# sanjita2911/CS230-distributed-machine-learning

Hardware: AMD Instinct MI355X
Metric: CV-fits/sec (whole node), 256-pt RF GridSearchCV on 1M×100 tabular (higher is better)
Workload: dtype fp32; 1 GPU; model=RandomForestClassifier, global_batch=20, parallelism=task1, rows=1000000, features=100, grid_points=256, cv=5, cands_per_rank_step=4

## Files before the change

### cs230_distributed_machine_learning_amd/csrc/kernels/forest.hip

```cpp
#include <hip/hip_runtime.h>
#include <stdint.h>
#include <math.h>
#include <type_traits>
#include <algorithm>
#include <stdio.h>
#include <stdlib.h>
#include <string.h>
#include "forest_common.h"
#include "wave_ops.h"

#ifndef DML_RPT_BLOCK
#define DML_RPT_BLOCK 1
#endif
#if DML_RPT_BLOCK < 1 || DML_RPT_BLOCK > 4
#error "DML_RPT_BLOCK must be 1..4"
#endif
#ifndef DML_BLOCK_NT
#define DML_BLOCK_NT 128
#endif
template <int MODE> constexpr int block_nt() { return MODE == 1 ? DML_BLOCK_NT : 256; }
#ifndef DML_NODES_WPE
#define DML_NODES_WPE 4
#endif
#ifndef DML_EVAL_NOINLINE
#define DML_EVAL_ATTR __attribute__((always_inline))
#else
#define DML_EVAL_ATTR
#endif
#ifndef DML_PART_U2
#define DML_PART_U2 4
#endif
#ifndef DML_KGL_LARGE
#define DML_KGL_LARGE 16
#endif
#ifndef DML_KGW_LARGE
#define DML_KGW_LARGE 32
#endif
#ifndef DML_LARGE_STASH
#define DML_LARGE_STASH 0
#endif
#ifndef DML_PART_KEEP
#define DML_PART_KEEP 2
#endif
#ifndef DML_NODES_WPE_WAVE
#define DML_NODES_WPE_WAVE 4
#endif
#ifndef DML_NODES_WPE_WAVE_MAX
#define DML_NODES_WPE_WAVE_MAX 8
#endif
#ifndef DML_KGMAX_BLOCK
#define DML_KGMAX_BLOCK 16
#endif
#ifndef DML_BLOCK_STREAM_ONLY
#define DML_BLOCK_STREAM_ONLY 1
#endif
#ifndef DML_NODES_WPE_REG
#define DML_NODES_WPE_REG 2
#endif
#ifndef DML_NODES_WPE_MC
#define DML_NODES_WPE_MC 2
#endif
#ifndef DML_SUB_SEG_REG
#define DML_SUB_SEG_REG 1
#endif
#ifndef DML_KGMAX_WAVE
#define DML_KGMAX_WAVE 4
#endif
#ifndef DML_WAVE_HIST32
#define DML_WAVE_HIST32 1
#endif
#ifndef DML_KGMAX_WAVE32
#define DML_KGMAX_WAVE32 5
#endif
#ifndef DML_ROW_WINDOWS
#define DML_ROW_WINDOWS 1
#endif
#ifndef DML_WAVE_WIN_ROWS
#define DML_WAVE_WIN_ROWS 4
#endif
#ifndef DML_GINI_PF
#define DML_GINI_PF 1
#endif
#ifndef DML_EVAL_PAIRS
#define DML_EVAL_PAIRS 0
#endif
#ifndef DML_WAVE_PREFETCH
#define DML_WAVE_PREFETCH 12
#endif
#ifndef DML_LARGE_NODE_FAST
#define DML_LARGE_NODE_FAST 1
#endif
#if DML_LARGE_NODE_FAST
// ... 880 lines not shown
    if (!PK && !c.packed) return pack_bin32(c.ycls[r.wd], boot_weight(s, r.wd));
    return pack_bin32((int)(r.wd >> (c.rbits + 4)), (r.wd >> c.rbits) & 15u);
  } else {
    return word_payload<MODE, PK>(c, s, ty, r.wd);
  }
}

template <int MODE>
__device__ __forceinline__ void hist_add_unit(typename HT<MODE>::T* hj, int b, const typename PLT<MODE>::T& pl,
                                              int wo) {
  if constexpr (MODE == 2) {
    atomicAdd((uint32_t*)hj + b, 1u);
    atomicAdd(&hj[wo + b], pl.wy);
  }
}

constexpr int kPackShift = 52;
constexpr unsigned long long kPackBias = 1ull << 39;
template <int MODE>
__device__ __forceinline__ void hist_add_packed(typename HT<MODE>::T* hj, int b, const typename PLT<MODE>::T& pl,
                                                int wo) {
  if constexpr (MODE == 2) atomicAdd(&hj[wo + b], (1ull << kPackShift) + ((unsigned long long)pl.wy + kPackBias));
}
__device__ __forceinline__ uint32_t pack_count(unsigned long long v) { return (uint32_t)(v >> kPackShift); }
__device__ __forceinline__ unsigned long long pack_wy(unsigned long long v) {
  return (v & ((1ull << kPackShift) - 1)) - ((v >> kPackShift) << 39);
}

template <int MODE>
__device__ __forceinline__ void hist_add_wy(typename HT<MODE>::T* hj, int b, const typename PLT<MODE>::T& pl,
                                            int wo) {
  if constexpr (MODE == 2) atomicAdd(&hj[wo + b], pl.wy);
}

template <int MODE, int RP = 3, class CT = typename HT<MODE>::T, class PL = typename PLT<MODE>::T>
__device__ __forceinline__ void hist_add(CT* hj, const Ctx& c, int b, const PL& pl) {
#ifdef DML_X2_ATOMIC
  if constexpr (MODE == 1) atomicAdd(&hj[b], (CT)(pl * (PL)((uint32_t)c.n >> 31)));
#endif
  if constexpr (MODE == 2) {
    atomicAdd(&hj[b], pl.wr);
    atomicAdd(&hj[256 + b], pl.wy);
    if (RP == 3) atomicAdd(&hj[512 + b], pl.wyy);
    return;
  }
  if constexpr (MODE == 0) {
    atomicAdd(&hj[(int)(uint32_t)pl * 256 + b], (uint32_t)(pl >> 32));
    atomicAdd(&hj[c.C * 256 + b], 1u);
  } else if constexpr (MODE == 1) {
    atomicAdd(&hj[b], (CT)pl);
  }
}

template <int NT, int MODE, int FC, bool H32 = false>
__global__ __launch_bounds__(NT) __attribute__((amdgpu_waves_per_eu(MODE == 2 ? DML_NODES_WPE_REG : (MODE == 0 ? DML_NODES_WPE_MC : (NT == 64 ? DML_NODES_WPE_WAVE : DML_NODES_WPE)), (MODE == 1 && NT == 64) ? DML_NODES_WPE_WAVE_MAX : 8))) void k_nodes(Ctx c, int tier, int set_cur,
                                                                                                   int pair_base, int stage_base) {
  static_assert(!H32 || (MODE == 1 && NT == 64), "the narrow word is the binary wave tier's");
  using CT = typename std::conditional<H32, uint32_t, typename HT<MODE>::T>::type;
  constexpr bool PK = FC >= 0;
  constexpr int NW = NT / 64;
  constexpr int RPT = NT == 64 ? 4 : DML_RPT_BLOCK;
  static_assert(RPT >= 1 && RPT <= 4, "RPT");
  static_assert(2 * RPT * (NT / 64) <= 32, "Scratch::wcnt too small for this NT x RPT");
  constexpr int KGMAX = NT == 64 ? (H32 ? DML_KGMAX_WAVE32 : DML_KGMAX_WAVE) : DML_KGMAX_BLOCK;
  extern __shared__ __attribute__((aligned(16))) unsigned char smem[];
  PH_BEGIN
  const OpenNode on = c.open[set_cur][tier][blockIdx.x];
  const NodeSpec s = spec_of<FC>(c, on.tree);
  const int tid = threadIdx.x, lane = tid & 63, wid = tid >> 6;
  const int d = c.d;
  const int KG = min(NT == 64 ? c.kg_wave : c.kg_block, KGMAX);
  const int slack = NT == 64 ? c.slack_wave : 0;
  const int span = hist_planes(MODE, c.CH) * 256;
  const FusedLayout FL = fused_layout(KG, span, (int)sizeof(CT), c.CH);
  CT* hist = (CT*)(smem + FL.hist);
  int16_t* feats = (int16_t*)(smem + FL.feats);
  double* rg = (double*)(smem + FL.rg);
  int* rb = (int*)(smem + FL.rb);
  int* rn = (int*)(smem + FL.rn);
  double* rleft = (double*)(smem + FL.rleft);
  double* rmid = (double*)(smem + FL.rmid);
  double* best_left = (double*)(smem + FL.best_left);
  double* pvs = (double*)(smem + FL.pvs);
  double* rvs = (double*)(smem + FL.rvs);
  Scratch* sc = (Scratch*)(smem + FL.sc);

  for (int i = tid; i < KG * span; i += NT) hist[i] = (CT)0;
  if (tid < c.VC) pvs[tid] = c.node_val[(int64_t)on.node * c.VC + tid];
  if (tid == 0) {
    sc->best_gain = -INFINITY; sc->best_feat = -1; sc->best_bin = -1;
    sc->nonconst = 0; sc->pos = 0; sc->first = 1; sc->last = 0; sc->best_j = -1;
    sc->best_pos = 1 << 30; sc->scr_n = 0;
    sc->W = c.tree_W[on.tree];
    sc->best_mid = 0.0;
    sc->lo = (FC < 0 && c.nbound) ? c.nbound[2 * (int64_t)on.node] : -INFINITY;
    sc->hi = (FC < 0 && c.nbound) ? c.nbound[2 * (int64_t)on.node + 1] : INFINITY;
  }
  const FeatPerm fp = feat_perm(on.key, d);
  const uint32_t* rows = c.rows_cur + on.start;
  const float* ty = tree_y(c, s);
  const int cnt = on.count;
  const bool reg_rows = (NT > 64 && DML_BLOCK_STREAM_ONLY) ? false : (H32 || cnt <= NT * RPT);
  uint32_t rrow[RPT], rbin[RPT];
  using PL = typename std::conditional<H32, uint32_t, typename PLT<MODE>::T>::type;
  PL rpl[RPT];
  PRaw rpr[RPT];
  auto load_rows = [&](int base) {
#pragma unroll
    for (int u = 0; u < RPT; ++u) {
      const int r = base + tid + NT * u;
      rrow[u] = r < cnt ? rows[r] : 0xFFFFFFFFu;
    }
  };
  auto fetch_rows = [&]() {
#pragma unroll
    for (int u = 0; u < RPT; ++u) rpr[u] = payload_fetch<MODE, PK>(c, ty, rrow[u]);
  };
  auto finish_rows = [&]() {
#pragma unroll
    for (int u = 0; u < RPT; ++u)
      rpl[u] = rrow[u] != 0xFFFFFFFFu ? payload_finish<MODE, PK, PL>(c, s, ty, rpr[u]) : PL{};
  };
  if (reg_rows) load_rows(0);
#pragma unroll
  for (int u = 0; u < RPT; ++u) rbin[u] = 0;
  __syncthreads();
  PH(0)
  if (reg_rows) fetch_rows();
  const int k = s.max_features;
  uint32_t pk[KGMAX];
  constexpr int KPRE = (NT == 64 && RPT == 4) ? DML_WAVE_PREFETCH : 0;
  uint32_t pre[KPRE > 0 ? KPRE : 1];
  int npre = 0;
  if constexpr (KPRE > 0) {
    if (reg_rows) {
      npre = min(KPRE, min(k + slack, d));
      if (DML_ROW_WINDOWS && DML_WAVE_WIN_ROWS > 0 && npre >= 8 && d <= 112 && (c.ld & 15) == 0 && c.ld >= 112 &&
          (((uintptr_t)c.Xb) & 15) == 0) {
        typedef uint32_t v32u __attribute__((ext_vector_type(32)));
        int fdw[KPRE], fsh[KPRE];
#pragma unroll
        for (int q = 0; q < KPRE; ++q) {
          const int f = __builtin_amdgcn_readfirstlane(q < npre ? feature_at(fp, q, d) : 0);
          fdw[q] = f >> 2;
          fsh[q] = (f & 3) * 8;
          pre[q] = 0u;
        }
        constexpr int WR = DML_WAVE_WIN_ROWS > 0 ? DML_WAVE_WIN_ROWS : 1;
#pragma unroll
        for (int u0 = 0; u0 < RPT; u0 += WR) {
          v32u w[WR];
#pragma unroll
          for (int uu = 0; uu < WR; ++uu) {
            const uint32_t r = rrow[u0 + uu];
// ... 30 lines not shown
      for (int q = 0; q < KPRE; ++q) {
        uint32_t v = 0;
#pragma unroll
        for (int u = 0; u < RPT; ++u) v |= raw[q][u] << (8 * u);
        pre[q] = v;
      }
      }
    }
  }
  if (reg_rows) finish_rows();
  while (true) {
    const int pos = __builtin_amdgcn_readfirstlane(sc->pos), nonconst = __builtin_amdgcn_readfirstlane(sc->nonconst);
    if (nonconst >= k || pos >= d) break;
    const int g = min(KG, min(k - nonconst + slack, d - pos));
    if (tid < g) feats[tid] = (int16_t)feature_at(fp, pos + tid, d);
    __syncthreads();
    PH(1)
    if (KPRE > 0 && reg_rows && pos + g <= npre) {
#pragma unroll
      for (int q = 0; q < (KPRE > 0 ? KPRE : 1); ++q) {
        if (q >= pos && q < pos + g) {
          CT* hj = hist + (q - pos) * span;
#pragma unroll
          for (int u = 0; u < RPT; ++u)
            if (rrow[u] != 0xFFFFFFFFu) hist_add<MODE>(hj, c, (int)((pre[q] >> (8 * u)) & 0xFFu), rpl[u]);
        }
      }
    } else
    if (!reg_rows && RPT == 1) {
      constexpr uint32_t INV = 0xFFFFFFFFu;
      auto run = [&](auto Gc) {
        constexpr int G = decltype(Gc)::value;
        int fj[G];
#pragma unroll
        for (int j = 0; j < G; ++j) fj[j] = __builtin_amdgcn_readfirstlane((int)feats[j < g ? j : 0]);
        auto row_at = [&](int r) -> uint32_t {
          const uint32_t v = rows[min(r, cnt - 1)];
          return r < cnt ? v : INV;
        };
        auto gather = [&](uint32_t r, uint32_t* b) {
          const uint8_t* xr = c.Xb + (int64_t)(r != INV ? (r & c.rmask) : 0u) * c.ld;
#pragma unroll
          for (int j = 0; j < G; ++j) b[j] = (uint32_t)xr[fj[j]];
#ifdef DML_X2_GATHER
#pragma unroll
          for (int j = 0; j < G; ++j) b[j] |= (uint32_t)xr[fj[j] + ((uint32_t)c.n >> 31)];
#endif
        };
        auto consume = [&](int base, bool valid, const uint32_t* b, const PRaw& pr) {
          if (NT > 64 && pos == 0 && valid) {
            uint32_t w4[4] = {0u, 0u, 0u, 0u};
#pragma unroll
            for (int j = 0; j < G && j < 16; ++j) w4[j >> 2] |= (j < g ? b[j] & 0xFFu : 0u) << (8 * (j & 3));
            *(uint4*)(c.bscr + (on.start + base + tid) * 16) = make_uint4(w4[0], w4[1], w4[2], w4[3]);
          }
          if (valid) {
            const PL pl = payload_finish<MODE, PK, PL>(c, s, ty, pr);
#pragma unroll
            for (int j = 0; j < G; ++j)
              if (j < g) hist_add<MODE>(hist + j * span, c, (int)b[j], pl);
          }
        };
        uint32_t rA = row_at(tid), rB = row_at(NT + tid);
        uint32_t bA[G], bB[G];
        gather(rA, bA);
        PRaw pA = payload_fetch<MODE, PK>(c, ty, rA), pB;
        bool vA = rA != INV, vB = false;
        for (int base = 0; base < cnt; base += 2 * NT) {
          rA = row_at(base + 2 * NT + tid);
          gather(rB, bB);
          pB = payload_fetch<MODE, PK>(c, ty, rB);
          vB = rB != INV;
          consume(base, vA, bA, pA);
          rB = row_at(base + 3 * NT + tid);
          gather(rA, bA);
          pA = payload_fetch<MODE, PK>(c, ty, rA);
          vA = rA != INV;
          consume(base + NT, vB, bB, pB);
        }
      };
      auto runw = [&](auto Gc) {
        constexpr int G = decltype(Gc)::value;
        typedef uint32_t v32u __attribute__((ext_vector_type(32)));
        int fdw[G], fsh[G];
#pragma unroll
        for (int j = 0; j < G; ++j) {
          const int f = __builtin_amdgcn_readfirstlane((int)feats[j < g ? j : 0]);
          fdw[j] = f >> 2;
          fsh[j] = (f & 3) * 8;
        }
        auto row_at = [&](int r) -> uint32_t {
          const uint32_t v = rows[min(r, cnt - 1)];
          return r < cnt ? v : INV;
        };
        auto load_win = [&](uint32_t r, v32u& w) {
          const uint4* xr = (const uint4*)(c.Xb + (int64_t)(r != INV ? (r & c.rmask) : 0u) * c.ld);
#pragma unroll
          for (int k = 0; k < 7; ++k) {
            const uint4 q = xr[k];
            w[4 * k] = q.x; w[4 * k + 1] = q.y; w[4 * k + 2] = q.z; w[4 * k + 3] = q.w;
          }
        };
        constexpr int NPK = (G + 3) / 4;
        auto extract = [&](const v32u& w, uint32_t* b) {
#pragma unroll
          for (int q = 0; q < NPK; ++q) b[q] = 0u;
#pragma unroll
          for (int j = 0; j < G; ++j) b[j >> 2] |= (j < g ? (w[fdw[j]] >> fsh[j]) & 0xFFu : 0u) << (8 * (j & 3));
        };
        auto consume = [&](int base, bool valid, const uint32_t* b, const PRaw& pr) {
          if (NT > 64 && pos == 0 && valid)
            *(uint4*)(c.bscr + (on.start + base + tid) * 16) =
                make_uint4(b[0], NPK > 1 ? b[NPK > 1 ? 1 : 0] : 0u, NPK > 2 ? b[NPK > 2 ? 2 : 0] : 0u,
                           NPK > 3 ? b[NPK > 3 ? 3 : 0] : 0u);
          if (valid) {
            const PL pl = payload_finish<MODE, PK, PL>(c, s, ty, pr);
#pragma unroll
            for (int j = 0; j < G; ++j)
              if (j < g) hist_add<MODE>(hist + j * span, c, (int)((b[j >> 2] >> (8 * (j & 3))) & 0xFFu), pl);
          }
        };
        v32u win;
        uint32_t bA[NPK], bB[NPK];
        uint32_t rA = row_at(tid), rB = row_at(NT + tid);
        load_win(rA, win);
        PRaw pA = payload_fetch<MODE, PK>(c, ty, rA), pB;
        extract(win, bA);
        bool vA = rA != INV, vB = false;
        for (int base = 0; base < cnt; base += 2 * NT) {
          load_win(rB, win);
          pB = payload_fetch<MODE, PK>(c, ty, rB);
          rA = row_at(base + 2 * NT + tid);
          consume(base, vA, bA, pA);
          extract(win, bB);
          vB = rB != INV;
          load_win(rA, win);
          pA = payload_fetch<MODE, PK>(c, ty, rA);
          rB = row_at(base + 3 * NT + tid);
          consume(base + NT, vB, bB, pB);
          extract(win, bA);
          vA = rA != INV;
        }
      };
      if (DML_ROW_WINDOWS && NT > 64 && pos == 0 && g >= 8 && d <= 112 && (c.ld & 15) == 0 && c.ld >= 112 &&
          (((uintptr_t)c.Xb) & 15) == 0) {
        switch (g) {
          case 8: runw(std::integral_constant<int, (8 < KGMAX ? 8 : KGMAX)>{}); break;
          case 9: runw(std::integral_constant<int, (9 < KGMAX ? 9 : KGMAX)>{}); break;
          case 10: runw(std::integral_constant<int, (10 < KGMAX ? 10 : KGMAX)>{}); break;
          case 11: runw(std::integral_constant<int, (11 < KGMAX ? 11 : KGMAX)>{}); break;
          case 12: runw(std::integral_constant<int, (12 < KGMAX ? 12 : KGMAX)>{}); break;
          default: runw(std::integral_constant<int, KGMAX>{}); break;
        }
      } else
      switch (g) {
#define DML_G_CASE(N) case N: run(std::integral_constant<int, (N < KGMAX ? N : KGMAX)>{}); break;
        DML_G_CASE(1) DML_G_CASE(2) DML_G_CASE(3) DML_G_CASE(4) DML_G_CASE(5) DML_G_CASE(6) DML_G_CASE(7)
        DML_G_CASE(8) DML_G_CASE(9) DML_G_CASE(10) DML_G_CASE(11) DML_G_CASE(12) DML_G_CASE(13) DML_G_CASE(14)
        DML_G_CASE(15)
#undef DML_G_CASE
        default: run(std::integral_constant<int, KGMAX>{}); break;
      }
    } else
    for (int base = 0; base < cnt; base += NT * RPT) {
      if (!reg_rows) { load_rows(base); fetch_rows(); }
      uint32_t bins[KGMAX][RPT];
#pragma unroll
      for (int j = 0; j < KGMAX; ++j) {
        if (j < g) {
          const int64_t f = feats[j];
#pragma unroll
          for (int u = 0; u < RPT; ++u)
            bins[j][u] = rrow[u] != 0xFFFFFFFFu ? (uint32_t)c.Xb[(int64_t)(rrow[u] & c.rmask) * c.ld + f] : 0u;
        }
      }
      if (!reg_rows) finish_rows();
#pragma unroll
      for (int j = 0; j < KGMAX; ++j) {
        if (j < g) {
          CT* hj = hist + j * span;
#pragma unroll
          for (int u = 0; u < RPT; ++u)
            if (rrow[u] != 0xFFFFFFFFu) hist_add<MODE>(hj, c, (int)bins[j][u], rpl[u]);
        }
      }
      if (NT > 64 && !reg_rows && pos == 0) {
#pragma unroll
        for (int u = 0; u < RPT; ++u)
          if (rrow[u] != 0xFFFFFFFFu) {
            uint32_t w4[4] = {0u, 0u, 0u, 0u};
#pragma unroll
            for (int j = 0; j < KGMAX && j < 16; ++j)
              if (j < g) w4[j >> 2] |= (bins[j][u] & 0xFFu) << (8 * (j & 3));
            *(uint4*)(c.bscr + (on.start + base + tid + NT * u) * 16) = make_uint4(w4[0], w4[1], w4[2], w4[3]);
          }
      }
      if (NT == 64 && !reg_rows && pos < 16) {
#pragma unroll
        for (int u = 0; u < RPT; ++u)
          if (rrow[u] != 0xFFFFFFFFu) {
            uint8_t* slot = c.bscr + (on.start + base + tid + NT * u) * 16;
#pragma unroll
            for (int j = 0; j < KGMAX; ++j)
              if (j < g && pos + j < 16) slot[pos + j] = (uint8_t)bins[j][u];
          }
      }
      if (reg_rows) {
#pragma unroll
        for (int j = 0; j < KGMAX; ++j)
        {
          uint32_t v = 0;
#pragma unroll
          for (int u = 0; u < RPT; ++u) v |= bins[j][u] << (8 * u);
          pk[j] = j < g ? v : 0u;
        }
      }
    }
    __syncthreads();
    PH(2)
    int j0 = wid;
#if !defined(DML_X2_EVAL) && DML_EVAL_PAIRS
    if constexpr (MODE == 1 && (DML_EVAL_PAIRS == 1 || (DML_EVAL_PAIRS == 2) == (NT == 64))) {
      const double* cw = tree_cw<FC>(c, on.tree);
      if (gini_pf_ok(s, cwk(cw, 0), cwk(cw, 1)))
        for (; j0 + NW < g; j0 += 2 * NW) {
          if (mono_of<FC>(c, s, feats[j0]) != 0 || mono_of<FC>(c, s, feats[j0 + NW]) != 0) break;
          eval_gini_pf<2, NW, CT>(hist + j0 * span, span, s, lane, rg + j0, rb + j0, rn + j0, rleft + j0 * c.CH, c.CH, true,
                              cwk(cw, 0), cwk(cw, 1));
          if (lane == 0) { rmid[j0] = 0.0; rmid[j0 + NW] = 0.0; }
        }
    }
#endif
    for (int j = j0; j < g; j += NW) {
#ifdef DML_X2_EVAL
      eval_feature<MODE, 3, CT>(hist + j * span, c.C, c.CH, s, lane, rg + j, rb + j, rn + j, rleft + j * c.CH, false,
                         tree_cw<FC>(c, on.tree), &c.rq, MonoQ{mono_of<FC>(c, s, feats[j]), sc->lo, sc->hi}, rmid + j);
      wave_lds_sync();
#endif
      eval_feature<MODE, 3, CT>(hist + j * span, c.C, c.CH, s, lane, rg + j, rb + j, rn + j, rleft + j * c.CH, true,
                         tree_cw<FC>(c, on.tree), &c.rq, MonoQ{mono_of<FC>(c, s, feats[j]), sc->lo, sc->hi}, rmid + j);
    }
    __syncthreads();
    PH(3)
    if (wid == 0) {
      const int nc0 = sc->nonconst;
      const bool isnc = lane < g && rn[lane] != 0;
      const uint64_t m = __ballot(isnc);
// ... 24 lines not shown
#pragma unroll
        for (int q = 0; q < (KPRE > 0 ? KPRE : 1); ++q)
          if (q == pos + bj) sel = pre[q];
      } else {
#pragma unroll
        for (int j = 0; j < KGMAX; ++j)
          if (j == bj) sel = pk[j];
      }
      if (bj >= 0)
#pragma unroll
        for (int u = 0; u < RPT; ++u) rbin[u] = (sel >> (8 * u)) & 0xFFu;
    }
  }
  if (tid == 0) {
    int base = pair_base + 2 * (int)blockIdx.x;
    NodeRec leaf; leaf.split = -1; leaf.left = -1;
    c.nodes[base] = leaf;
    c.nodes[base + 1] = leaf;
    if (!(sc->best_feat >= 0 && accept_split_v(c, s, pvs, sc->W, best_left))) {
      base = -1;
      c.stage[2 * (stage_base + (int64_t)blockIdx.x)].tier = -1;
      c.stage[2 * (stage_base + (int64_t)blockIdx.x) + 1].tier = -1;
    } else {
      {
        double* lv = c.node_val + (int64_t)base * c.VC;
        for (int q = 0; q < c.VC; ++q) {
          rvs[q] = pvs[q] - best_left[q];
          lv[q] = best_left[q];
          lv[c.VC + q] = rvs[q];
        }
        NodeRec rec; rec.split = pack_split(sc->best_feat, sc->best_bin); rec.left = base;
        c.nodes[on.node] = rec;
        mono_children<FC>(c, on.node, base, mono_of<FC>(c, s, sc->best_feat), sc->best_mid);
      }
    }
    sc->base = base;
    sc->nl = base >= 0 ? (int)best_left[c.CH - 1] : 0;
  }
  __syncthreads();
  PH(5)
  const int base = sc->base;
  if (base < 0) { PH_END(NT == 64 ? 0 : 1) return; }
  const int feat = sc->best_feat, bin = sc->best_bin, nl = sc->nl;
  constexpr int RT = NT > 64 ? 64 : 1;
  if (tid == 0)
    stage_child<FC>(c, s, on.tree, base, on.start, nl, on.depth + 1, child_key(on.key, 0),
                2 * (stage_base + (int64_t)blockIdx.x), best_left);
  if (tid == RT)
    stage_child<FC>(c, s, on.tree, base + 1, on.start + nl, cnt - nl, on.depth + 1, child_key(on.key, 1),
                2 * (stage_base + (int64_t)blockIdx.x) + 1, rvs);
#ifdef DML_X2_PART
  for (int rep_ = 0; rep_ < 2; ++rep_) {
#endif
  if (NT > 64 && !reg_rows && cnt <= 128 * NT && (size_t)((cnt + 63) / 64) * 12 <= (size_t)KG * span * sizeof(CT)) {
    uint64_t* lflag = (uint64_t*)hist;
    int* loff = (int*)(lflag + ((cnt + 63) / 64));
    const int ngrp = (cnt + 63) / 64;
    const int bjs = __builtin_amdgcn_readfirstlane((sc->best_pos < sc->scr_n) ? sc->best_pos : -1);
    const int fsplit = __builtin_amdgcn_readfirstlane(feat), bsplit = __builtin_amdgcn_readfirstlane(bin);
    constexpr int U = 4;
    constexpr int KR = DML_PART_KEEP;
    static_assert(DML_PART_U2 == U, "pass 2 walks the positions of pass 1");
    uint32_t rk[KR > 0 ? KR : 1][U];
#pragma unroll
    for (int q = 0; q < (KR > 0 ? KR : 1); ++q)
#pragma unroll
      for (int u = 0; u < U; ++u) rk[q][u] = 0u;
    for (int p0 = 0, q = 0; p0 < cnt; p0 += U * NT, ++q) {
      uint32_t bv[U];
#pragma unroll
      for (int u = 0; u < U; ++u) {
        const int p = min(p0 + u * NT + tid, cnt - 1);
        const uint32_t r = (KR > 0 || bjs < 0) ? rows[p] : 0u;
        if (bjs >= 0) {
          bv[u] = c.bscr[(on.start + p) * 16 + bjs];
        } else {
          bv[u] = c.Xb[(int64_t)(r & c.rmask) * c.ld + fsplit];
        }
#pragma unroll
        for (int qq = 0; qq < KR; ++qq)
          if (qq == q) rk[qq][u] = r;
      }
#pragma unroll
      for (int u = 0; u < U; ++u) {
        const int p = p0 + u * NT + tid;
        const uint64_t m = __ballot(p < cnt && (int)bv[u] <= bsplit);
        if (lane == 0 && p - lane < cnt) lflag[(p - lane) >> 6] = m;
      }
    }
    __syncthreads();
    {
      const int g0 = 2 * tid, g1 = 2 * tid + 1;
      const int c0 = g0 < ngrp ? __popcll(lflag[g0]) : 0, c1 = g1 < ngrp ? __popcll(lflag[g1]) : 0;
      const int incl = wave::incl_scan<int>(c0 + c1);
      if (lane == 63) sc->wcnt[wid] = incl;
      __syncthreads();
      int wbase = 0;
      for (int w = 0; w < wid; ++w) wbase += sc->wcnt[w];
      const int ex = wbase + incl - (c0 + c1);
      if (g0 < ngrp) loff[g0] = ex;
      if (g1 < ngrp) loff[g1] = ex + c0;
    }
    __syncthreads();
    constexpr int U2 = DML_PART_U2;
    for (int p0 = tid, q = 0; p0 < cnt; p0 += U2 * NT, ++q) {
      uint32_t rr[U2];
      if (q < KR) {
#pragma unroll
        for (int qq = 0; qq < KR; ++qq)
          if (qq == q)
#pragma unroll
            for (int u = 0; u < U2; ++u) rr[u] = rk[qq][u];
      } else {
#pragma unroll
        for (int u = 0; u < U2; ++u) rr[u] = rows[min(p0 + u * NT, cnt - 1)];
      }
#pragma unroll
      for (int u = 0; u < U2; ++u) {
        const int p = p0 + u * NT;
        if (p >= cnt) break;
        const int q = p >> 6;
        const uint64_t m = lflag[q];
        const int lft = __popcll(m & ((1ull << (p & 63)) - 1ull));
        const bool left = (m >> (p & 63)) & 1ull;
        const int l0 = loff[q];
        c.rows_next[on.start + (left ? l0 + lft : nl + (q * 64 - l0) + ((p & 63) - lft))] = rr[u];
      }
    }
  } else {
  uint32_t* out = c.rows_next + on.start;
  int baseL = 0, baseR = 0;
  constexpr uint32_t INVR = 0xFFFFFFFFu;
  auto prow = [&](int r) -> uint32_t { return r < cnt ? rows[r] : INVR; };
  const int bj_scr = (!reg_rows && sc->best_pos < sc->scr_n) ? sc->best_pos : -1;
  auto pbin = [&](int p, uint32_t r) -> uint32_t {
    if (r == INVR) return 0u;
    if (bj_scr >= 0) return (uint32_t)c.bscr[(on.start + p) * 16 + bj_scr];
    return (uint32_t)c.Xb[(int64_t)(r & c.rmask) * c.ld + feat];
  };
  uint32_t nrow = INVR, nbin = 0, frow = INVR;
  if (!reg_rows && RPT == 1) {
    rrow[0] = prow(tid);
    rbin[0] = pbin(tid, rrow[0]);
    nrow = prow(NT + tid);
  }
  for (int cb = 0; cb < cnt; cb += NT * RPT) {
    if (!reg_rows) {
      if constexpr (RPT == 1) {
        nbin = pbin(cb + NT + tid, nrow);
        frow = prow(cb + 2 * NT + tid);
      } else {
        load_rows(cb);
#pragma unroll
        for (int u = 0; u < RPT; ++u)
          rbin[u] = rrow[u] == 0xFFFFFFFFu ? 0u
                  : bj_scr >= 0 ? (uint32_t)c.bscr[(on.start + cb + tid + NT * u) * 16 + bj_scr]
                                : (uint32_t)c.Xb[(int64_t)(rrow[u] & c.rmask) * c.ld + feat];
      }
    }
    uint64_t ml[RPT], mr[RPT];
#pragma unroll
    for (int u = 0; u < RPT; ++u) {
      const bool valid = rrow[u] != 0xFFFFFFFFu;
      const bool left = valid && (int)rbin[u] <= bin;
      ml[u] = __ballot(left);
      mr[u] = __ballot(valid && !left);
    }
    int offL[RPT], offR[RPT], totL = 0, totR = 0;
    if constexpr (NW == 1) {
#pragma unroll
      for (int u = 0; u < RPT; ++u) {
        offL[u] = totL; offR[u] = totR;
        totL += __popcll(ml[u]); totR += __popcll(mr[u]);
      }
    } else {
      if (lane == 0)
#pragma unroll
        for (int u = 0; u < RPT; ++u) {
          sc->wcnt[u * NW + wid] = __popcll(ml[u]);
          sc->wcnt[RPT * NW + u * NW + wid] = __popcll(mr[u]);
        }
      __syncthreads();
#pragma unroll
      for (int u = 0; u < RPT; ++u) {
        int l = 0, r = 0, lb = 0, rbb = 0;
        for (int w = 0; w < NW; ++w) {
          const int cl = sc->wcnt[u * NW + w], cr = sc->wcnt[RPT * NW + u * NW + w];
          if (w < wid) { lb += cl; rbb += cr; }
          l += cl; r += cr;
        }
        offL[u] = totL + lb; offR[u] = totR + rbb;
        totL += l; totR += r;
      }
      __syncthreads();
    }
#pragma unroll
    for (int u = 0; u < RPT; ++u) {
      const bool valid = rrow[u] != 0xFFFFFFFFu;
      if (!valid) continue;
      if ((int)rbin[u] <= bin) out[baseL + offL[u] + lane_prefix(ml[u])] = rrow[u];
      else out[nl + baseR + offR[u] + lane_prefix(mr[u])] = rrow[u];
    }
    baseL += totL; baseR += totR;
    if (!reg_rows && RPT == 1) { rrow[0] = nrow; rbin[0] = nbin; nrow = frow; }
  }
  }
#ifdef DML_X2_PART
  }
#endif
// ... 1926 lines not shown
  t_lane = lane;
  return kLanes;
}

__global__ void k_test_wave_prims(const uint32_t* in, uint32_t* out) {
  const int lane = threadIdx.x;
  const uint32_t v = in[blockIdx.x * 64 + lane];
  uint32_t* o = out + (size_t)blockIdx.x * 64 * 11;
  o[0 * 64 + lane] = wave::bitonic64(v, lane);
  o[1 * 64 + lane] = wave::incl_scan<uint32_t>(v);
  o[2 * 64 + lane] = wave::xor32<1>(v, lane);
  o[3 * 64 + lane] = wave::xor32<2>(v, lane);
  o[4 * 64 + lane] = wave::xor32<4>(v, lane);
  o[5 * 64 + lane] = wave::xor32<8>(v, lane);
  o[6 * 64 + lane] = wave::xor32<16>(v, lane);
  o[7 * 64 + lane] = wave::xor32<32>(v, lane);
  double g = (double)(v % 97u);
  int idx = lane;
  wave::argmax(g, idx, lane);
  o[8 * 64 + lane] = (uint32_t)idx;
  o[9 * 64 + lane] = (uint32_t)wave::shift_down1<int>((int)v, lane, -1);
  o[10 * 64 + lane] = (uint32_t)wave::min_u64(((uint64_t)v << 32) | (uint32_t)lane, lane);
}

struct PredictArgs;
extern "C" int dml_forest_predict_fit(const PredictArgs* a, int32_t f, hipStream_t st);

extern "C" {

int dml_forest_phase_stats(unsigned long long* out) {
#ifdef DML_PHASE_PROF
  if (hipMemcpyFromSymbol(out, HIP_SYMBOL(g_phase), sizeof(unsigned long long) * 32) != hipSuccess) return 1;
  unsigned long long z[32] = {0};
  if (hipMemcpyToSymbol(HIP_SYMBOL(g_phase), z, sizeof(z)) != hipSuccess) return 1;
  return 0;
#else
  (void)out;
  return 2;
#endif
}

int dml_test_wave_prims(const uint32_t* in, uint32_t* out, int64_t nblocks, hipStream_t st) {
  k_test_wave_prims<<<(unsigned)nblocks, 64, 0, st>>>(in, out);
  return hipGetLastError() == hipSuccess ? 0 : 1;
}

const char* dml_forest_last_error(int* line) {
  if (line) *line = g_last_err_line;
  return hipGetErrorString(g_last_err);
}

int dml_forest_wave_hist32() { return DML_WAVE_HIST32 != 0 ? 1 : 0; }
int dml_forest_large_stash() { return DML_LARGE_STASH != 0 ? 1 : 0; }
int dml_forest_sizeof_treespec() { return (int)sizeof(TreeSpec); }
int dml_forest_sizeof_args() { return (int)sizeof(ForestArgs); }
int dml_forest_sizeof_node() { return (int)sizeof(NodeRec); }

int64_t dml_forest_workspace_bytes(const ForestArgs* a) {
  Layout L = plan(a);
  return (int64_t)(L.total + align_up((size_t)a->rows_total * 4, 256));
}

int dml_forest_count(ForestArgs* a, hipStream_t st) {
  Ctx c{};
  c.n = (int)a->n; c.roles = (const uint8_t*)a->roles; c.specs = (const TreeSpec*)a->specs;
  c.active_count = (int32_t*)a->active_count;
  HIP_OK(hipMemsetAsync(c.active_count, 0, a->T * 4, st));
  dim3 grid((unsigned)((a->n + 1023) / 1024), (unsigned)((a->T + kCntG - 1) / kCntG));
  k_count_active<<<grid, 256, 0, st>>>(c, (int)a->T);
  HIP_OK(hipGetLastError());
  return 0;
}

}

template <int MODE>
static int build_impl(ForestArgs* a, hipStream_t st) {
  constexpr bool REG = MODE == 2;
  constexpr int GM = MODE == 2 ? 2 : 0;
  constexpr int FCX = REG ? kMSE : kGini;
  Layout L = plan(a);
  if ((size_t)a->workspace_bytes < (size_t)dml_forest_workspace_bytes(a)) return 2;
  Ctx c = make_ctx(a, L);
  const bool fast = a->fast_crit == FCX + 1 && c.packed;
  const bool big = MODE == 1 && a->bigsub_max > 0;
  if (big && (a->bigsub_max > 256 || a->wave_max > a->bigsub_max || a->sub_cache_d <= 0 || a->mono || a->n_classes != 2))
    return 12;
  if (big) c.bigsub_max = (int)a->bigsub_max;
  const size_t lds_big = big ? big_layout((int)a->bigsub_max, (int)a->sub_cache_d).total + 16 : 0;
  uint32_t* rows_a = (uint32_t*)(((unsigned char*)a->workspace) + L.total);
  c.rows_cur = rows_a;
  int32_t* h = pinned_counters();
  if (!h) return 3;
  const bool reg = REG;
  if (!reg && (a->n_classes < 1 || a->n_classes > kMaxClasses)) return 5;
  if (a->d > 32767) return 6;

  HIP_OK(hipMemsetAsync(c.counters, 0, kNumCounters * 4, st));
  HIP_OK(hipMemsetAsync(c.cursors, 0, a->T * 4, st));
  HIP_OK(hipMemsetAsync(c.node_val, 0, (size_t)a->T * c.VC * 8, st));
  if (reg) HIP_OK(hipMemsetAsync(c.rsum, 0, (size_t)a->T * 3 * 8, st));
  k_init_counters<<<1, 1, 0, st>>>(c);
  dim3 gfill((unsigned)((a->n + 1023) / 1024), (unsigned)a->T);
  if (reg) k_fill_active<true><<<gfill, 256, 0, st>>>(c);
  else k_fill_active<false><<<gfill, 256, 0, st>>>(c);
  k_roots<<<(unsigned)((a->T + 255) / 256), 256, 0, st>>>(c);
// ... 271 lines not shown
```

### cs230_distributed_machine_learning_amd/csrc/kernels/forest_common.h

```cpp
#pragma once
#include <stdint.h>

#if defined(__HIPCC__)
#include <hip/hip_runtime.h>
#define DML_HD __host__ __device__ __forceinline__
#define DML_HDM __host__ __device__ __forceinline__
#else
#include <math.h>
#define DML_HD static inline
#define DML_HDM inline
#endif

namespace dml {

constexpr int kBins = 256;
constexpr int kPoisTable = 12;
constexpr int kMaxClasses = 64;

enum Criterion : int32_t { kGini = 0, kEntropy = 1, kMSE = 2, kPoisson = 3, kMAE = 4, kFriedman = 5 };

struct TreeSpec {
  uint64_t seed;
  int32_t split;
  int32_t fit;
// ... 78 lines not shown
  p.m3 = ((uint32_t)h3 | 1u) & p.mask; p.a3 = (uint32_t)(h3 >> 32) & p.mask;
  if (p.mask == 1u) { p.m1 = p.m2 = p.m3 = 1u; }
  return p;
}

DML_HD uint32_t feat_perm_step(const FeatPerm& p, uint32_t x) {
  x = (x * p.m1 + p.a1) & p.mask;
  x ^= x >> p.sh;
  x = (x * p.m2 + p.a2) & p.mask;
  x ^= x >> p.sh;
  x = (x * p.m3 + p.a3) & p.mask;
  x ^= x >> p.sh;
  return x;
}

DML_HD int feature_at(const FeatPerm& p, int k, int d) {
  uint32_t x = feat_perm_step(p, (uint32_t)k);
  while (x >= (uint32_t)d) x = feat_perm_step(p, x);
  return (int)x;
}

constexpr uint64_t kPackMask21 = (1ull << 21) - 1ull;
constexpr int kPackMaxRows = 131072;
DML_HD uint64_t pack_bin(int cls, uint32_t w) {
  return (cls == 0 ? (uint64_t)w : ((uint64_t)w << 21)) | (1ull << 42);
}

constexpr int kRowWeightBits = 4;
constexpr int kPack32MaxRows = 255;
constexpr int kPack32MaxWeight = 1 << kRowWeightBits;
constexpr uint32_t kPack32Mask12 = (1u << 12) - 1u;
static_assert(kPoisTable < kPack32MaxWeight, "a bootstrap weight must fit the row word's weight field");
static_assert(kPack32MaxWeight * kPack32MaxRows < 4096, "a 255-row node's class weight must fit 12 bits");
static_assert(kPack32MaxRows < 256, "a 255-row node's row count must fit 8 bits");
DML_HD uint32_t pack_bin32(int cls, uint32_t w) { return (cls == 0 ? w : (w << 12)) | (1u << 24); }
DML_HD uint32_t bin32_w0(uint32_t v) { return v & kPack32Mask12; }
DML_HD uint32_t bin32_w1(uint32_t v) { return (v >> 12) & kPack32Mask12; }
DML_HD uint32_t bin32_rows(uint32_t v) { return v >> 24; }

template <class CT>
DML_HD uint32_t pk_w0(CT v) {
  if constexpr (sizeof(CT) == 8) return (uint32_t)((uint64_t)v & kPackMask21);
  else return bin32_w0((uint32_t)v);
}
template <class CT>
DML_HD uint32_t pk_w1(CT v) {
  if constexpr (sizeof(CT) == 8) return (uint32_t)(((uint64_t)v >> 21) & kPackMask21);
  else return bin32_w1((uint32_t)v);
}
template <class CT>
DML_HD uint32_t pk_rows(CT v) {
  if constexpr (sizeof(CT) == 8) return (uint32_t)((uint64_t)v >> 42);
  else return bin32_rows((uint32_t)v);
}

#if defined(__HIPCC__)
#pragma clang fp contract(off)
#endif

DML_HD double dlog2(double x) {
  int e;
#if defined(__HIP_DEVICE_COMPILE__)
  double m = ::frexp(x, &e);
#else
  double m = frexp(x, &e);
#endif
  if (m < 0.70710678118654752440) {
    m = m * 2.0;
    e -= 1;
  }
  const double s = (m - 1.0) / (m + 1.0);
  const double s2 = s * s;
  double p = 1.0 / 21.0;
  p = p * s2 + 1.0 / 19.0;
  p = p * s2 + 1.0 / 17.0;
  p = p * s2 + 1.0 / 15.0;
  p = p * s2 + 1.0 / 13.0;
  p = p * s2 + 1.0 / 11.0;
  p = p * s2 + 1.0 / 9.0;
  p = p * s2 + 1.0 / 7.0;
  p = p * s2 + 1.0 / 5.0;
  p = p * s2 + 1.0 / 3.0;
  p = p * s2 + 1.0;
  return (double)e + (2.0 * s * p) * 1.44269504088896340736;
}

struct ClsAcc {
  double w, sq, clogc;
  bool ent;
  DML_HDM void init(int crit) { w = 0.0; sq = 0.0; clogc = 0.0; ent = crit == kEntropy; }
  DML_HDM void add(double c) {
    w += c;
    sq += c * c;
    if (ent && c > 0.0) clogc += c * dlog2(c);
  }
};

DML_HD double cls_impurity(const ClsAcc& a, int crit) {
  if (a.w <= 0.0) return 0.0;
  if (crit == kEntropy) return dlog2(a.w) - a.clogc / a.w;
  return 1.0 - a.sq / (a.w * a.w);
}

DML_HD double cls_proxy(const ClsAcc& l, const ClsAcc& r, int crit) {
  if (crit == kEntropy) return (l.clogc - l.w * dlog2(l.w)) + (r.clogc - r.w * dlog2(r.w));
  return (l.sq * r.w + r.sq * l.w) / (l.w * r.w);
// ... 246 lines not shown
```

### cs230_distributed_machine_learning_amd/csrc/runtime/forest_cpu.cpp

```cpp
#include <stdint.h>
#include <string.h>
#include <math.h>
#include <vector>
#include <algorithm>
#include "../kernels/forest_common.h"

namespace dml {

struct CpuTree {
  std::vector<NodeRec> nodes;
  std::vector<double> vals;
};

struct CpuForest {
  int T = 0, VC = 0;
  std::vector<CpuTree> trees;
};

struct Data {
  const uint8_t* Xb; int64_t ld; int n, d, C, CH, VC, is_reg;
  const int32_t* ycls; const float* yreg; const uint8_t* roles;
  int64_t ystride;
  const double* cw;
  const int8_t* mono;
// ... 342 lines not shown
  }
  D.mono = mono;
  D.ystride = ystride;
  D.cw = cw;
  D.Xb = Xb; D.ld = ld; D.n = (int)n; D.d = (int)d; D.is_reg = (int)is_reg;
  D.C = is_reg ? 1 : (int)n_classes;
  D.CH = is_reg ? 4 : (int)n_classes + 1;
  D.VC = is_reg ? 3 : (int)n_classes;
  D.ycls = ycls; D.yreg = yreg; D.roles = roles;
  CpuForest* F = new CpuForest();
  F->T = (int)T;
  F->VC = D.VC;
  F->trees.resize(T);
#pragma omp parallel for schedule(dynamic, 1)
  for (int64_t t = 0; t < T; ++t) build_tree(D, specs[t], t, F->trees[t]);
  return F;
}

void* dml_cpu_forest_build(const uint8_t* Xb, int64_t ld, int64_t n, int64_t d, const int32_t* ycls,
                           const float* yreg, int64_t n_classes, int64_t is_reg, const uint8_t* roles,
                           const TreeSpec* specs, int64_t T, int64_t ystride, const double* cw) {
  int e1 = 0, e2 = 0;
  if (is_reg) {
    int64_t targets = 1;
    if (ystride > 0)
      for (int64_t t = 0; t < T; ++t) targets = std::max<int64_t>(targets, (int64_t)specs[t].target + 1);
    std::vector<int64_t> cnt((size_t)targets * kExpBins, 0);
    for (int64_t t = 0; t < targets; ++t)
      for (int64_t i = 0; i < n; ++i) {
        const float y = yreg[(ystride > 0 ? t * ystride : 0) + i];
        int k = 0;
        if (y != 0.0f) frexp((double)y, &k);
        cnt[(size_t)t * kExpBins + (y != 0.0f ? k + kExpOff : 0)]++;
      }
    reg_exponents_counts(cnt.data(), targets, e1, e2);
  }
  return dml_cpu_forest_build_mono(Xb, ld, n, d, ycls, yreg, n_classes, is_reg, roles, specs, T, ystride, cw,
                                   nullptr, e1, e2);
}

void dml_reg_exponents(const int64_t* cnt, int64_t targets, int32_t* out) {
  int e1, e2;
  reg_exponents_counts(cnt, targets, e1, e2);
  out[0] = e1; out[1] = e2;
}

uint32_t dml_pack_bin32(int32_t cls, uint32_t w) { return pack_bin32(cls, w); }
void dml_bin32_fields(uint32_t v, uint32_t* out) {
  out[0] = bin32_w0(v); out[1] = bin32_w1(v); out[2] = bin32_rows(v);
  if (pk_w0<uint32_t>(v) != out[0] || pk_w1<uint32_t>(v) != out[1] || pk_rows<uint32_t>(v) != out[2]) out[2] = ~0u;
}
void dml_pack32_limits(int32_t* out) { out[0] = kPack32MaxRows; out[1] = kPack32MaxWeight; out[2] = kPoisTable; }

int64_t dml_cpu_forest_num_nodes(void* h) {
  CpuForest* F = (CpuForest*)h;
  int64_t s = 0;
  for (auto& t : F->trees) s += (int64_t)t.nodes.size();
  return s;
}

void dml_cpu_forest_export(void* h, NodeRec* nodes, double* vals) {
  CpuForest* F = (CpuForest*)h;
  int64_t next = F->T;
  for (int t = 0; t < F->T; ++t) {
    const CpuTree& tr = F->trees[t];
    const int64_t base = next;
    auto gidx = [&](int64_t local) { return local == 0 ? (int64_t)t : base + local - 1; };
    for (size_t i = 0; i < tr.nodes.size(); ++i) {
      NodeRec r = tr.nodes[i];
      if (r.left >= 0) r.left = (int32_t)gidx(r.left);
      const int64_t g = gidx((int64_t)i);
      nodes[g] = r;
      memcpy(vals + g * F->VC, tr.vals.data() + i * F->VC, sizeof(double) * F->VC);
    }
    next += (int64_t)tr.nodes.size() - 1;
  }
}

void dml_cpu_forest_apply(const uint8_t* Xb, int64_t ld, int64_t n, const NodeRec* nodes, int32_t t0, int32_t T,
                          int32_t* leaf) {
#pragma omp parallel for collapse(2) schedule(static)
  for (int32_t t = 0; t < T; ++t)
    for (int64_t r = 0; r < n; ++r) {
      const uint8_t* xr = Xb + r * ld;
      int node = t0 + t;
      NodeRec nr = nodes[node];
      while (nr.split >= 0) {
        node = nr.left + (xr[nr.split >> 8] > (nr.split & 255) ? 1 : 0);
        nr = nodes[node];
      }
      leaf[(int64_t)t * n + r] = node;
    }
}

void dml_cpu_forest_prune(NodeRec* nodes, const double* vals, int64_t VC, int32_t C, int32_t is_reg,
                          const TreeSpec* specs, const int32_t* limit, int32_t T, int32_t* leaves) {
  std::vector<FrontierEnt> heap;
  for (int32_t t = 0; t < T; ++t) {
    if (limit[t] <= 0) {
      if (leaves) leaves[t] = -1;
      continue;
    }
    heap.resize((size_t)limit[t]);
    const int n = best_first_prune(nodes, vals, VC, C, is_reg != 0, specs[t].criterion, t, limit[t], heap.data());
    if (leaves) leaves[t] = n;
  }
// ... 107 lines not shown
```

### cs230_distributed_machine_learning_amd/utils/native.py

```python
from __future__ import annotations

import ctypes
import os
import threading

import numpy as np

from .. import build as _build

_lock = threading.Lock()
_hip = None
_cpu = None

c_i64 = ctypes.c_int64
c_i32 = ctypes.c_int32
c_vp = ctypes.c_void_p

POIS_TABLE = 12

TREESPEC_DTYPE = np.dtype(
    [
        ("seed", "<u8"),
        ("split", "<i4"),
        ("fit", "<i4"),
# ... 149 lines not shown
            lib.dml_forest_predict_fit.argtypes = [ctypes.POINTER(PredictArgs), c_i32, c_vp]
            lib.dml_scores.restype = c_i32
            lib.dml_scores.argtypes = [ctypes.POINTER(ScoreArgs), c_vp]
            lib.dml_bin.restype = c_i32
            lib.dml_bin.argtypes = [c_vp, c_i64, c_i64, c_vp, c_vp, c_i64, c_vp]
            _register_optional(lib)
            _hip = lib
        return _hip


def _register_optional(lib) -> None:
    table = {
        "dml_lr_link_grad": (c_i32, [c_vp, c_i64, c_i64, c_vp, c_vp, c_vp, c_vp, c_vp, c_vp, c_vp, c_i64, c_vp, c_i64,
                                     c_vp, c_vp, c_vp]),
        "dml_lr_predict": (c_i32, [c_vp, c_i64, c_vp, c_vp, c_i64, c_vp, c_vp, c_vp, c_i64, c_vp, c_vp]),
        "dml_knn_l2_mfma": (c_i32, [c_vp, c_i64, c_i32, c_vp, c_vp, c_i64, c_i64, c_vp, c_vp, c_vp, c_i64, c_i32, c_vp,
                                    c_vp, c_vp]),
        "dml_knn": (c_i32, [c_vp, c_vp, c_i64, c_i64, c_vp, c_vp, c_vp, c_i64, c_i32, ctypes.c_float, c_i32, c_vp,
                            c_vp, c_vp]),
        "dml_knn_qpw": (c_i32, []),
        "dml_forest_apply": (c_i32, [c_vp, c_i64, c_i64, c_vp, c_i32, c_i32, c_vp, c_vp]),
        "dml_forest_prune": (c_i32, [c_vp, c_vp, c_i64, c_i32, c_i32, c_vp, c_vp, c_i32, c_i32, c_vp, c_i64, c_vp, c_vp]),
        "dml_svm_sizeof_prob": (c_i32, []),
        "dml_forest_set_lane": (c_i32, [c_i32]),
        "dml_forest_refine": (c_i32, [c_vp, c_i64, c_i64, c_i64, c_vp, c_i64, c_vp, c_i32, c_vp, c_vp, c_vp, c_vp,
                                      c_vp]),
        "dml_svm_smo_split": (c_i32, [c_vp, c_i64, c_vp, c_i64, c_i32, c_i32, c_vp, c_vp, c_vp, c_vp, c_vp, c_vp,
                                      c_vp, c_vp, c_vp, c_i64, c_vp, c_i32, c_vp]),
        "dml_svm_split_limits": (c_i32, [c_vp, c_vp, c_vp]),
        "dml_svm_smo": (c_i32, [c_vp, c_i64, c_vp, c_i64, c_vp, c_vp, c_vp, c_vp, c_vp, c_vp, c_i64, c_vp]),
        "dml_split_moments": (c_i32, [c_vp, c_i64, c_vp, c_vp, c_vp, c_i64, c_i64, c_i32, c_vp, c_i64, c_vp]),
        "dml_lr_mfma_tile": (c_i32, []),
        "dml_lr_mfma_fwd": (c_i32, [ctypes.POINTER(LrFwdArgs), c_vp]),
        "dml_lr_mfma_grad": (c_i32, [ctypes.POINTER(LrGradArgs), c_vp]),
        "dml_lr_v3_row_tile": (c_i32, []),
        "dml_lr_mfma_fwd3": (c_i32, [ctypes.POINTER(LrFwdArgs), c_vp]),
        "dml_lr_mfma_grad3": (c_i32, [ctypes.POINTER(LrGradArgs), c_vp]),
        "dml_split_hilo": (c_i32, [c_vp, c_i64, c_i64, c_i64, c_vp, c_vp, c_i64, c_i32, c_vp, c_vp]),
        "dml_lr_sizeof_fwd_args": (c_i32, []),
        "dml_lr_sizeof_grad_args": (c_i32, []),
        "dml_dp_sizeof_args": (c_i32, []),
        "dml_dp_sizeof_slot": (c_i32, []),
        "dml_dp_step": (c_i32, [c_vp, c_i32, c_vp]),
        "dml_gb_sizeof_stage_args": (c_i32, []),
        "dml_gb_sizeof_grad_args": (c_i32, []),
        "dml_gb_stage": (c_i32, [ctypes.POINTER(GbStageArgs), c_vp]),
        "dml_gb_grad": (c_i32, [ctypes.POINTER(GbGradArgs), c_vp]),
        "dml_gb_huber_delta": (c_i32, [ctypes.POINTER(GbGradArgs), c_vp]),
        "dml_gb_stage_phase": (c_i32, [ctypes.POINTER(GbStageArgs), c_vp]),
        "dml_gb_sel_step": (c_i32, [ctypes.POINTER(GbStageArgs), c_i32, c_i32, c_vp]),
        "dml_gb_fit_sel_step": (c_i32, [ctypes.POINTER(GbGradArgs), c_i32, c_i32, c_vp]),
        "dml_exp_hist": (c_i32, [c_vp, c_i64, c_i64, c_i64, c_vp, c_vp, c_vp]),
        "dml_forest_release_scratch": (c_i32, []),
        "dml_mae_sizeof_args": (c_i32, []),
        "dml_mae_sizeof_open": (c_i32, []),
        "dml_mae_sizeof_res": (c_i32, []),
        "dml_mae_count": (c_i32, [ctypes.POINTER(MaeArgs), c_vp]),
        "dml_mae_build": (c_i32, [ctypes.POINTER(MaeArgs), c_vp]),
    }
    for name, (res, args) in table.items():
        fn = getattr(lib, name, None)
        if fn is not None:
            fn.restype = res
            fn.argtypes = args
    if getattr(lib, "dml_gb_sizeof_stage_args", None) is not None:
        if (lib.dml_gb_sizeof_stage_args() != ctypes.sizeof(GbStageArgs)
                or lib.dml_gb_sizeof_grad_args() != ctypes.sizeof(GbGradArgs)):
            raise RuntimeError("GBRT stage argument layout mismatch between HIP library and Python")
    if getattr(lib, "dml_mae_sizeof_args", None) is not None and lib.dml_mae_sizeof_args() != ctypes.sizeof(MaeArgs):
        raise RuntimeError("MAE builder argument layout mismatch between HIP library and Python")
    if getattr(lib, "dml_lr_sizeof_fwd_args", None) is not None:
        if (lib.dml_lr_sizeof_fwd_args() != ctypes.sizeof(LrFwdArgs)
                or lib.dml_lr_sizeof_grad_args() != ctypes.sizeof(LrGradArgs)):
            raise RuntimeError("LR MFMA argument layout mismatch between HIP library and Python")


def hip_error(lib=None) -> str:
    lib = lib or hip_lib()
    line = c_i32(0)
    msg = lib.dml_forest_last_error(ctypes.byref(line))
    return f"{msg.decode() if msg else '?'} (forest.hip:{line.value})"


def ptr(t) -> int:
    if t is None:
        return 0
    if isinstance(t, np.ndarray):
        return int(t.ctypes.data)
    return int(t.data_ptr())


def stream_handle(device=None) -> int:
    import torch

    return int(torch.cuda.current_stream(device).cuda_stream)


def poisson_cdf_table(lam: float) -> np.ndarray:
    import math

    out = np.empty(POIS_TABLE, dtype=np.uint64)
    p = math.exp(-lam)
    cdf = 0.0
    for j in range(POIS_TABLE):
        cdf += p
        p *= lam / (j + 1)
# ... 3 lines not shown
```

Baseline: 28.43 CV-fits/s.

## Stash block-tier bins in per-word planes and extend LDS partition to all counts

Changes the per-node bin stash from a 16-byte interleaved row record to planar 4-byte words per group of four features. Partition reads of the best feature become coalesced 32-bit loads instead of strided byte loads, and planes for unused feature groups are not written. It also allows the LDS flag-based partition for any node count that fits, using a multi-group-per-thread scan. The risk is more store instructions per row when many planes are written, and a longer serial scan loop for large nodes.

```diff
diff --git a/cs230_distributed_machine_learning_amd/csrc/kernels/forest.hip b/cs230_distributed_machine_learning_amd/csrc/kernels/forest.hip
--- a/cs230_distributed_machine_learning_amd/csrc/kernels/forest.hip
+++ b/cs230_distributed_machine_learning_amd/csrc/kernels/forest.hip
@@ -38,6 +38,12 @@
 #endif
 #ifndef DML_LARGE_STASH
 #define DML_LARGE_STASH 0
+#endif
+#ifndef DML_BLOCK_STASH_PLANES
+#define DML_BLOCK_STASH_PLANES 1
+#endif
+#ifndef DML_BLOCK_PART_ALL
+#define DML_BLOCK_PART_ALL 1
 #endif
 #ifndef DML_PART_KEEP
 #define DML_PART_KEEP 2
@@ -1024,6 +1030,10 @@
   }
 }
 
+__device__ __forceinline__ uint32_t* plane_word(uint8_t* plane, int p) {
+  return (uint32_t*)(plane + 4u * (uint32_t)p);
+}
+
 template <int NT, int MODE, int FC, bool H32 = false>
 __global__ __launch_bounds__(NT) __attribute__((amdgpu_waves_per_eu(MODE == 2 ? DML_NODES_WPE_REG : (MODE == 0 ? DML_NODES_WPE_MC : (NT == 64 ? DML_NODES_WPE_WAVE : DML_NODES_WPE)), (MODE == 1 && NT == 64) ? DML_NODES_WPE_WAVE_MAX : 8))) void k_nodes(Ctx c, int tier, int set_cur,
                                                                                                    int pair_base, int stage_base) {
@@ -1072,6 +1082,9 @@
   const uint32_t* rows = c.rows_cur + on.start;
   const float* ty = tree_y(c, s);
   const int cnt = on.count;
+  constexpr bool PLANES = NT > 64 && DML_BLOCK_STASH_PLANES != 0;
+  uint8_t* const stash0 = c.bscr + stash_plane_base(on.start, cnt, 0);
+  auto plane = [&](int w) -> uint8_t* { return stash0 + 4 * (int64_t)cnt * w; };
   const bool reg_rows = (NT > 64 && DML_BLOCK_STREAM_ONLY) ? false : (H32 || cnt <= NT * RPT);
   uint32_t rrow[RPT], rbin[RPT];
   using PL = typename std::conditional<H32, uint32_t, typename PLT<MODE>::T>::type;
@@ -1208,7 +1221,12 @@
             uint32_t w4[4] = {0u, 0u, 0u, 0u};
 #pragma unroll
             for (int j = 0; j < G && j < 16; ++j) w4[j >> 2] |= (j < g ? b[j] & 0xFFu : 0u) << (8 * (j & 3));
-            *(uint4*)(c.bscr + (on.start + base + tid) * 16) = make_uint4(w4[0], w4[1], w4[2], w4[3]);
+            if constexpr (PLANES) {
+#pragma unroll
+              for (int w = 0; w < stash_planes(G); ++w) *plane_word(plane(w), base + tid) = w4[w];
+            } else {
+              *(uint4*)(c.bscr + (on.start + base + tid) * 16) = make_uint4(w4[0], w4[1], w4[2], w4[3]);
+            }
           }
           if (valid) {
             const PL pl = payload_finish<MODE, PK, PL>(c, s, ty, pr);
@@ -1265,10 +1283,16 @@
           for (int j = 0; j < G; ++j) b[j >> 2] |= (j < g ? (w[fdw[j]] >> fsh[j]) & 0xFFu : 0u) << (8 * (j & 3));
         };
         auto consume = [&](int base, bool valid, const uint32_t* b, const PRaw& pr) {
-          if (NT > 64 && pos == 0 && valid)
-            *(uint4*)(c.bscr + (on.start + base + tid) * 16) =
-                make_uint4(b[0], NPK > 1 ? b[NPK > 1 ? 1 : 0] : 0u, NPK > 2 ? b[NPK > 2 ? 2 : 0] : 0u,
-                           NPK > 3 ? b[NPK > 3 ? 3 : 0] : 0u);
+          if (NT > 64 && pos == 0 && valid) {
+            if constexpr (PLANES) {
+#pragma unroll
+              for (int w = 0; w < stash_planes(G); ++w) *plane_word(plane(w), base + tid) = b[w];
+            } else {
+              *(uint4*)(c.bscr + (on.start + base + tid) * 16) =
+                  make_uint4(b[0], NPK > 1 ? b[NPK > 1 ? 1 : 0] : 0u, NPK > 2 ? b[NPK > 2 ? 2 : 0] : 0u,
+                             NPK > 3 ? b[NPK > 3 ? 3 : 0] : 0u);
+            }
+          }
           if (valid) {
             const PL pl = payload_finish<MODE, PK, PL>(c, s, ty, pr);
 #pragma unroll
@@ -1348,7 +1372,13 @@
 #pragma unroll
             for (int j = 0; j < KGMAX && j < 16; ++j)
               if (j < g) w4[j >> 2] |= (bins[j][u] & 0xFFu) << (8 * (j & 3));
-            *(uint4*)(c.bscr + (on.start + base + tid + NT * u) * 16) = make_uint4(w4[0], w4[1], w4[2], w4[3]);
+            if constexpr (PLANES) {
+#pragma unroll
+              for (int w = 0; w < stash_planes(KGMAX); ++w)
+                if (4 * w < g) *plane_word(plane(w), base + tid + NT * u) = w4[w];
+            } else {
+              *(uint4*)(c.bscr + (on.start + base + tid + NT * u) * 16) = make_uint4(w4[0], w4[1], w4[2], w4[3]);
+            }
           }
       }
       if (NT == 64 && !reg_rows && pos < 16) {
@@ -1479,12 +1509,15 @@
 #ifdef DML_X2_PART
   for (int rep_ = 0; rep_ < 2; ++rep_) {
 #endif
-  if (NT > 64 && !reg_rows && cnt <= 128 * NT && (size_t)((cnt + 63) / 64) * 12 <= (size_t)KG * span * sizeof(CT)) {
+  if (NT > 64 && !reg_rows && (DML_BLOCK_PART_ALL || cnt <= 128 * NT) &&
+      (size_t)((cnt + 63) / 64) * 12 <= (size_t)KG * span * sizeof(CT)) {
     uint64_t* lflag = (uint64_t*)hist;
     int* loff = (int*)(lflag + ((cnt + 63) / 64));
     const int ngrp = (cnt + 63) / 64;
     const int bjs = __builtin_amdgcn_readfirstlane((sc->best_pos < sc->scr_n) ? sc->best_pos : -1);
     const int fsplit = __builtin_amdgcn_readfirstlane(feat), bsplit = __builtin_amdgcn_readfirstlane(bin);
+    uint8_t* const bpl = plane(max(bjs, 0) >> 2);
+    const int bsh = 8 * (max(bjs, 0) & 3);
     constexpr int U = 4;
     constexpr int KR = DML_PART_KEEP;
     static_assert(DML_PART_U2 == U, "pass 2 walks the positions of pass 1");
@@ -1500,7 +1533,8 @@
         const int p = min(p0 + u * NT + tid, cnt - 1);
         const uint32_t r = (KR > 0 || bjs < 0) ? rows[p] : 0u;
         if (bjs >= 0) {
-          bv[u] = c.bscr[(on.start + p) * 16 + bjs];
+          if constexpr (PLANES) bv[u] = (*plane_word(bpl, p) >> bsh) & 0xFFu;
+          else bv[u] = c.bscr[(on.start + p) * 16 + bjs];
         } else {
           bv[u] = c.Xb[(int64_t)(r & c.rmask) * c.ld + fsplit];
         }
@@ -1516,7 +1550,20 @@
       }
     }
     __syncthreads();
-    {
+    if constexpr (DML_BLOCK_PART_ALL) {
+      const int gpt = (ngrp + NT - 1) / NT, gb = gpt * tid;
+      int tot = 0;
+      for (int i = 0; i < gpt; ++i) tot += gb + i < ngrp ? __popcll(lflag[gb + i]) : 0;
+      const int incl = wave::incl_scan<int>(tot);
+      if (lane == 63) sc->wcnt[wid] = incl;
+      __syncthreads();
+      int ex = incl - tot;
+      for (int w = 0; w < wid; ++w) ex += sc->wcnt[w];
+      for (int i = 0; i < gpt && gb + i < ngrp; ++i) {
+        loff[gb + i] = ex;
+        ex += __popcll(lflag[gb + i]);
+      }
+    } else {
       const int g0 = 2 * tid, g1 = 2 * tid + 1;
       const int c0 = g0 < ngrp ? __popcll(lflag[g0]) : 0, c1 = g1 < ngrp ? __popcll(lflag[g1]) : 0;
       const int incl = wave::incl_scan<int>(c0 + c1);
@@ -1562,7 +1609,10 @@
   const int bj_scr = (!reg_rows && sc->best_pos < sc->scr_n) ? sc->best_pos : -1;
   auto pbin = [&](int p, uint32_t r) -> uint32_t {
     if (r == INVR) return 0u;
-    if (bj_scr >= 0) return (uint32_t)c.bscr[(on.start + p) * 16 + bj_scr];
+    if (bj_scr >= 0) {
+      if constexpr (PLANES) return (*plane_word(plane(bj_scr >> 2), p) >> (8 * (bj_scr & 3))) & 0xFFu;
+      else return (uint32_t)c.bscr[(on.start + p) * 16 + bj_scr];
+    }
     return (uint32_t)c.Xb[(int64_t)(r & c.rmask) * c.ld + feat];
   };
   uint32_t nrow = INVR, nbin = 0, frow = INVR;
@@ -1581,7 +1631,7 @@
 #pragma unroll
         for (int u = 0; u < RPT; ++u)
           rbin[u] = rrow[u] == 0xFFFFFFFFu ? 0u
-                  : bj_scr >= 0 ? (uint32_t)c.bscr[(on.start + cb + tid + NT * u) * 16 + bj_scr]
+                  : bj_scr >= 0 ? pbin(cb + tid + NT * u, rrow[u])
                                 : (uint32_t)c.Xb[(int64_t)(rrow[u] & c.rmask) * c.ld + feat];
       }
     }
@@ -3614,6 +3664,7 @@
 
 int dml_forest_wave_hist32() { return DML_WAVE_HIST32 != 0 ? 1 : 0; }
 int dml_forest_large_stash() { return DML_LARGE_STASH != 0 ? 1 : 0; }
+int dml_forest_block_stash_planes() { return DML_BLOCK_STASH_PLANES != 0 ? 1 : 0; }
 int dml_forest_sizeof_treespec() { return (int)sizeof(TreeSpec); }
 int dml_forest_sizeof_args() { return (int)sizeof(ForestArgs); }
 int dml_forest_sizeof_node() { return (int)sizeof(NodeRec); }
diff --git a/cs230_distributed_machine_learning_amd/csrc/kernels/forest_common.h b/cs230_distributed_machine_learning_amd/csrc/kernels/forest_common.h
--- a/cs230_distributed_machine_learning_amd/csrc/kernels/forest_common.h
+++ b/cs230_distributed_machine_learning_amd/csrc/kernels/forest_common.h
@@ -154,6 +154,13 @@
 DML_HD uint32_t pk_rows(CT v) {
   if constexpr (sizeof(CT) == 8) return (uint32_t)((uint64_t)v >> 42);
   else return bin32_rows((uint32_t)v);
+}
+
+constexpr int kStashSlot = 16;
+DML_HD constexpr int stash_planes(int g) { return ((g < kStashSlot ? g : kStashSlot) + 3) >> 2; }
+DML_HD int64_t stash_plane_base(int64_t start, int cnt, int w) { return kStashSlot * start + 4 * (int64_t)cnt * w; }
+DML_HD int64_t stash_plane_byte(int64_t start, int cnt, int p, int q) {
+  return stash_plane_base(start, cnt, q >> 2) + 4 * (int64_t)p + (q & 3);
 }
 
 #if defined(__HIPCC__)
diff --git a/cs230_distributed_machine_learning_amd/csrc/runtime/forest_cpu.cpp b/cs230_distributed_machine_learning_amd/csrc/runtime/forest_cpu.cpp
--- a/cs230_distributed_machine_learning_amd/csrc/runtime/forest_cpu.cpp
+++ b/cs230_distributed_machine_learning_amd/csrc/runtime/forest_cpu.cpp
@@ -418,6 +418,13 @@
 }
 void dml_pack32_limits(int32_t* out) { out[0] = kPack32MaxRows; out[1] = kPack32MaxWeight; out[2] = kPoisTable; }
 
+int32_t dml_stash_planes(int32_t g) { return stash_planes(g); }
+int64_t dml_stash_plane_base(int64_t start, int32_t cnt, int32_t w) { return stash_plane_base(start, cnt, w); }
+void dml_stash_plane_bytes(int64_t start, int32_t cnt, int32_t g, int64_t* out) {
+  for (int32_t p = 0; p < cnt; ++p)
+    for (int32_t q = 0; q < g; ++q) out[(int64_t)p * g + q] = stash_plane_byte(start, cnt, p, q);
+}
+
 int64_t dml_cpu_forest_num_nodes(void* h) {
   CpuForest* F = (CpuForest*)h;
   int64_t s = 0;
diff --git a/cs230_distributed_machine_learning_amd/utils/native.py b/cs230_distributed_machine_learning_amd/utils/native.py
--- a/cs230_distributed_machine_learning_amd/utils/native.py
+++ b/cs230_distributed_machine_learning_amd/utils/native.py
@@ -225,6 +225,7 @@
         "dml_gb_fit_sel_step": (c_i32, [ctypes.POINTER(GbGradArgs), c_i32, c_i32, c_vp]),
         "dml_exp_hist": (c_i32, [c_vp, c_i64, c_i64, c_i64, c_vp, c_vp, c_vp]),
         "dml_forest_release_scratch": (c_i32, []),
+        "dml_forest_block_stash_planes": (c_i32, []),
         "dml_mae_sizeof_args": (c_i32, []),
         "dml_mae_sizeof_open": (c_i32, []),
         "dml_mae_sizeof_res": (c_i32, []),
```

Result: faster. 28.79 CV-fits/s (median of 6 runs) (+1.2%).
